# hidasib/GRU4Rec

Measured on AMD Instinct MI355X. Metric: mini-batches/sec (gru4rec.py:661), RSC15-shaped batch=128 n_sample=2048 BPR-max, higher is better.
Workload: dtype f32

## Files before the change

gru4rec_amd/csrc/g4r_eval_kernels.cuh:

```cuda
#pragma once
#include "g4r_step_kernels.cuh"

#define SC_BM 128
#define SC_KC 128

template <int TN, bool COUNT = false>
__global__ __launch_bounds__(256) void k_score_all(const DevModel* __restrict__ mp, const float* h, int mrows, const int* item_idx,
                                                   long long n_sel, float* out, long long ldo, int apply_act,
                                                   int* cnt = nullptr, long long col_begin = 0, const int* tie_col = nullptr,
                                                   unsigned tie_ctr = 0) {
    extern __shared__ __attribute__((aligned(16))) float smem[];
    const DevModel& m = *mp;
    const int tid = threadIdx.x, lane = tid & 63, wid = tid >> 6, li = lane & 15, lg = lane >> 4;
    const int D = m.Dtop;
    const int ldk = SC_KC + 2;
    float* sA = smem;
    float* sB = sA + SC_BM * ldk;
    int* sItem = reinterpret_cast<int*>(sB + TN * ldk);
    const long long n0 = (long long)blockIdx.x * TN;
    const int rbase = blockIdx.y * SC_BM;
    if (tid < TN) {
        const long long n = n0 + tid;
        int item = -1;
        if (n < n_sel) item = item_idx ? item_idx[n] : (int)n;
// ... 182 lines not shown

__global__ void k_selftest_mfma32(const float* A, const float* Bm, float* C, int K) {
    const int lane = threadIdx.x & 63, l32 = lane & 31, lh = lane >> 5;
    f32x16 acc;
    for (int j = 0; j < 16; ++j) acc[j] = 0.f;
    for (int k = 0; k < K; k += 2) acc = mfma32(A[l32 * K + k + lh], Bm[(k + lh) * 32 + l32], acc);
    for (int r = 0; r < 16; ++r) C[(8 * (r >> 2) + 4 * lh + (r & 3)) * 32 + l32] = acc[r];
}

template __global__ void k_sparse_update<1, false>(const DevModel*, StepState*, int);
template __global__ void k_sparse_update<1, true>(const DevModel*, StepState*, int);
template __global__ void k_sparse_update<2, false>(const DevModel*, StepState*, int);
template __global__ void k_sparse_update<2, true>(const DevModel*, StepState*, int);
template __global__ void k_sparse_update_generic<1>(const DevModel*, StepState*, int, int);
template __global__ void k_sparse_update_generic<2>(const DevModel*, StepState*, int, int);
template __global__ void k_loss_rows<false, 0, 1>(const DevModel*, StepState*);
template __global__ void k_loss_rows<false, 0, 4>(const DevModel*, StepState*);
template __global__ void k_loss_rows<false, 1, 1>(const DevModel*, StepState*);
template __global__ void k_loss_rows<false, 1, 4>(const DevModel*, StepState*);
template __global__ void k_loss_rows<false, 2, 1>(const DevModel*, StepState*);
template __global__ void k_loss_rows<false, 2, 4>(const DevModel*, StepState*);
template __global__ void k_loss_rows<false, 3, 1>(const DevModel*, StepState*);
template __global__ void k_loss_rows<false, 3, 4>(const DevModel*, StepState*);
template __global__ void k_loss_rows<true, 0, 4>(const DevModel*, StepState*);
template __global__ void k_loss_rows<true, 1, 4>(const DevModel*, StepState*);
template __global__ void k_loss_rows<true, 2, 4>(const DevModel*, StepState*);
template __global__ void k_loss_rows<true, 3, 4>(const DevModel*, StepState*);
template __global__ void k_sparse_update<4, false>(const DevModel*, StepState*, int);
template __global__ void k_sparse_update<4, true>(const DevModel*, StepState*, int);
template __global__ void k_sparse_update_generic<4>(const DevModel*, StepState*, int, int);
template __global__ void k_update<1, 32, false>(const DevModel*, StepState*, const DenseTile*, int, int);
template __global__ void k_update<1, 32, true>(const DevModel*, StepState*, const DenseTile*, int, int);
template __global__ void k_update<2, 32, false>(const DevModel*, StepState*, const DenseTile*, int, int);
template __global__ void k_update<2, 32, true>(const DevModel*, StepState*, const DenseTile*, int, int);
template __global__ void k_dense_grad<32>(const DevModel*, StepState*, const DenseTile*);
template __global__ void k_score_fwd<GT_BN, GT_BK>(const DevModel*, StepState*);
template __global__ void k_score_fwd<32, 64>(const DevModel*, StepState*);
template __global__ void k_score_fwd<64, 32, T2_BK>(const DevModel*, StepState*);
template __global__ void k_score_fwd<64, 32, 3>(const DevModel*, StepState*);
template __global__ void k_score_bwd<32, GT_BK>(const DevModel*, StepState*, int, int, int, int);
template __global__ void k_score_bwd<64, 64>(const DevModel*, StepState*, int, int, int, int);
template __global__ void k_gru_p1<GT_BN, P1_BK>(const DevModel*, StepState*, int, int, int, GruFwdPredict);
// ... 8 lines not shown
```

gru4rec_amd/csrc/g4r_host_debug.hpp:

```cpp
int g4r_get_debug(g4r_model* m, const char* name, float* host, int64_t count) {
    if (!m || !name || !host) return fail("null argument");
    HIPCHK(hipSetDevice(m->cfg.device));
    DevModel& d = m->dm;
    const StepKernels& k = m->kern;
    std::string s(name);
    const float* p = nullptr; int64_t n = 0;
    int l = 0;
    if (!s.empty() && isdigit((unsigned char)s.back())) { l = s.back() - '0'; s.pop_back(); }
    if (l >= d.n_layers) return fail("layer out of range");
    const int64_t bd = (int64_t)d.B * d.D[l];
    if (s == "scores") { p = d.Sc; n = (int64_t)d.B * d.ldSc; }
    else if (s == "dSx") { p = d.dSx + (size_t)((m->gstep - 1) & d.defer_mask) * (size_t)d.dSx_stride; n = (int64_t)d.B * d.Ein; }
    else if (s == "dSy") { p = d.dSy + (size_t)((m->gstep - 1) & d.defer_mask) * (size_t)d.dSy_stride; n = (int64_t)d.ldSc * d.Dtop; }
    else if (s == "dSBy") { p = d.dSBy + (size_t)((m->gstep - 1) & d.defer_mask) * (size_t)d.dSBy_stride; n = d.ldSc; }
    else if (s == "defer_stats") {
        if (count < 4) return fail("count");
        double rows = 0, bias = 0;
        if (m->defer_on) {
            std::vector<unsigned> st(2048);
            HIPCHK(hipStreamSynchronize(m->stream));
            HIPCHK(hipMemcpy(st.data(), d.dstat, st.size() * sizeof(unsigned), hipMemcpyDeviceToHost));
            for (size_t i = 0; i < st.size(); i += 2) { rows += st[i]; bias += st[i + 1]; }
        }
        host[0] = (float)rows; host[1] = (float)bias; host[2] = m->defer_on ? 1.f : 0.f; host[3] = (float)(d.defer_mask + 1);
// ... 10 lines not shown
        host[1] = (m->sim_valid[0] || m->sim_valid[1]) ? 1.f : 0.f; host[2] = (float)m->sim_builds;
        return 0;
    }
    else if (s == "continue_steps") {
        if (count < 2) return fail("count");
        host[0] = (float)m->ro_calls; host[1] = (float)m->ro_steps;
        return 0;
    }
    else if (s == "events_launches") {
        if (count < 4) return fail("count");
        host[0] = (float)m->ev_steps; host[1] = (float)m->ev_scans; host[2] = (float)m->ev_launches; host[3] = (float)m->ev_pieces;
        return 0;
    }
    else if (s == "dhpart") { p = d.dhpart; n = (int64_t)d.ksplit * d.B * d.Dtop; }
    else if (s == "lossrow") { p = d.lossrow; n = d.B; }
    else if (s == "hd") { p = d.hd[l]; n = bd; }
    else if (s == "r") { p = d.r[l]; n = bd; }
    else if (s == "z") { p = d.z[l]; n = bd; }
    else if (s == "c") { p = d.c[l]; n = bd; }
    else if (s == "Hr") { p = d.Hr[l]; n = bd; }
    else if (s == "dV") { p = d.dV[l]; n = bd * 3; }
    else if (s == "dyl") { p = d.dyl[l]; n = bd; }
    else if (s == "Hprev") { p = d.H[l][(m->gstep + 1) & 1]; n = bd; }
    else if (s == "occ_idx") { p = (const float*)d.occ_idx; n = d.R; }
    else if (s == "own_pos") {
        if (!d.own_pos) return fail("no owner table (k_update_l not chosen, or G4R_OWNER_SCAN=1)");
        p = (const float*)(d.own_pos + (m->own_window ? (size_t)m->own_last * d.R * 16 : (size_t)0)); n = 16 * (int64_t)d.R;
    }
    else if (s == "own_pos_ring") { if (!d.own_pos) return fail("no owner table (k_update_l not chosen, or G4R_OWNER_SCAN=1)"); p = (const float*)d.own_pos; n = (int64_t)G4R_OWN_SLOTS * 16 * d.R; }
    else if (s == "owner_window") { if (count < 1) return fail("count"); host[0] = (m->own_window && k.update == UP_LEAN) ? 1.f : 0.f; return 0; }
// ... 63 lines not shown
}

int g4r_debug_loss_rows(g4r_model* m, float* scores, int64_t count, int32_t M, float* lossrow) {
    if (!m || !scores || !lossrow) return fail("null argument");
    DevModel& d = m->dm;
    if (count != (int64_t)d.B * d.ldSc) return fail("size mismatch for the score rows: expected " + std::to_string((int64_t)d.B * d.ldSc));
    if (M < 1 || M > d.B) return fail("M outside [1, batch_size]");
    HIPCHK(hipSetDevice(m->cfg.device));
    HIPCHK(hipStreamSynchronize(m->stream));
    StepState saved, mine;
    HIPCHK(hipMemcpy(&saved, (const void*)d.st, sizeof(saved), hipMemcpyDeviceToHost));
    HIPCHK(hipMemcpy((void*)d.Sc, scores, (size_t)count * sizeof(float), hipMemcpyHostToDevice));
    mine = saved;
    mine.M_b = M;
    HIPCHK(hipMemcpy((void*)d.st, &mine, sizeof(mine), hipMemcpyHostToDevice));
    StepLauncher lk(m, nullptr);
    launch_loss_rows(lk, dim3(d.B));
    hipError_t e = hipGetLastError();
    if (e == hipSuccess) e = hipStreamSynchronize(m->stream);
    const hipError_t r = hipMemcpy((void*)d.st, &saved, sizeof(saved), hipMemcpyHostToDevice);
    if (e != hipSuccess) return fail(std::string("k_loss_rows: ") + hipGetErrorString(e));
    if (r != hipSuccess) return fail(std::string("step state: ") + hipGetErrorString(r));
    HIPCHK(hipMemcpy(scores, (const void*)d.Sc, (size_t)count * sizeof(float), hipMemcpyDeviceToHost));
    HIPCHK(hipMemcpy(lossrow, (const void*)d.lossrow, (size_t)d.B * sizeof(float), hipMemcpyDeviceToHost));
    return 0;
}

int g4r_debug_gumbel(g4r_model* m, uint64_t seed, uint32_t row_id, uint32_t step, const int32_t* items, int64_t n, float* out) {
    if (!m || !items || !out) return fail("null argument");
    if (n < 1) return fail("n must be positive");
    for (int64_t p = 0; p < n; ++p)
        if (items[p] < 0) return fail("item index out of range");
    HIPCHK(hipSetDevice(m->cfg.device));
    CallTemps tmp(m);
    int* d_it = nullptr;
// ... 132 lines not shown
```

gru4rec_amd/csrc/g4r_host_step.hpp:

```cpp
extern "C++" {
struct StepLauncher {
    g4r_model* m;
    hipStream_t s;
    std::vector<EvRec>* recs;
    size_t evi = 0;
    int kn = -1;
    hipEvent_t ev_a = nullptr, ev_b = nullptr;
    StepLauncher(g4r_model* m_, std::vector<EvRec>* recs_) : m(m_), s(m_->stream), recs(recs_) {}
    void use(int kn_, hipEvent_t a, hipEvent_t b) { kn = kn_; ev_a = a; ev_b = b; }
    void open(int kn_) {
        if (m->sw.trace) { fprintf(stderr, "[g4r] launch %s\n", KN_NAMES[kn_]); fflush(stderr); }
        use(kn_, nullptr, nullptr);
        if (!recs) return;
        while (m->evs.size() < evi + 2) { hipEvent_t e; (void)hipEventCreate(&e); m->evs.push_back(e); }
        use(kn_, m->evs[evi], m->evs[evi + 1]);
        evi += 2;
        recs->push_back(EvRec{kn_, ev_a, ev_b});
    }
    bool skipped() const { return m->sw.skip_kn && kn >= 0 && ((m->sw.skip_kn >> kn) & 1ull); }
    template <class... P, class... A>
    void launch(void (*kern)(P...), dim3 grid, dim3 block, size_t smem, A... a) {
        if (skipped()) return;
        if (ev_a) hipExtLaunchKernelGGL(kern, grid, block, (unsigned)smem, s, ev_a, ev_b, 0, static_cast<P>(a)...);
        else hipLaunchKernelGGL(kern, grid, block, smem, s, static_cast<P>(a)...);
    }
    void close() {
        if (!m->sw.trace) return;
        hipError_t e = hipStreamSynchronize(s);
        fprintf(stderr, "[g4r] done   %s: %s\n", KN_NAMES[kn], hipGetErrorString(e));
        fflush(stderr);
    }
};
}

static void launch_loss_rows(StepLauncher& lk, dim3 grid) {
    g4r_model* m = lk.m;
    lk.launch(loss_rows_kernel(m->kern), grid, dim3(LOSS_T), m->smem_loss, (const DevModel*)m->d_dm, (StepState*)m->dm.st);
}

static inline bool update_merged(const g4r_model* m, const StepLauncher& lk) { return m->kern.update != UP_SPLIT && !(lk.recs && m->profile_split); }

static void gru_forward(g4r_model* m, StepLauncher& lk, int l) {
    const DevModel& d = m->dm;
    const StepKernels& k = m->kern;
    const int B = d.B, first = l == 0 ? 1 : 0;
    const DevModel* dmp = (const DevModel*)m->d_dm;
    StepState* stp = (StepState*)d.st;
    const GruFwdPredict nopa = {};
    if (k.fwd[l] == FWD_LEAN) {
        const dim3 g(cdiv(d.D[l], 16), cdiv(B, 16));
        const LeanV& v = m->h_leanV[l];
        const LeanH& h = m->h_leanH[l];
// ... 257 lines not shown
        HIPCHK(hipMemcpyAsync(Hc, m->d_tmpH, (size_t)B * W * sizeof(float), hipMemcpyDeviceToDevice, m->stream));
    }
    return 0;
}
static int between_steps(g4r_model* m, int64_t t, size_t* ci) {
    while (*ci < m->compact_steps.size() && m->compact_steps[*ci] == t) { if (apply_compaction(m, (int64_t)*ci)) return -1; ++*ci; }
    if (m->dm.ns > 0 && !m->store_frozen && m->gstep > 0 && m->gstep % m->gl == 0) {
        if (refill_store(m)) return -1;
        hipLaunchKernelGGL(k_restage_inputs, dim3(1), dim3(512), 0, m->stream, (const DevModel*)m->d_dm, (StepState*)m->dm.st);
    }
    return 0;
}

#define G4R_GRAPH_STEPS 16
#define G4R_GRAPH_STEPS_SMALL 4
static int capture_steps(g4r_model* m, int n, hipStreamCaptureMode cmode, hipGraphExec_t* out) {
    hipGraph_t graph = nullptr;
    HIPCHK(hipStreamBeginCapture(m->stream, cmode));
    int rc = 0;
    for (int i = 0; i < n && !rc; ++i) rc = whole_step(m, i);
    hipError_t e = hipStreamEndCapture(m->stream, &graph);
    if (rc || e != hipSuccess || !graph) {
        if (graph) (void)hipGraphDestroy(graph);
        (void)hipGetLastError();
        if (!rc) fail(std::string("graph capture: ") + hipGetErrorString(e));
        return -1;
    }
    e = hipGraphInstantiate(out, graph, nullptr, nullptr, 0);
    (void)hipGraphDestroy(graph);
    if (e != hipSuccess) { *out = nullptr; (void)hipGetLastError(); return fail(std::string("graph instantiate: ") + hipGetErrorString(e)); }
    return 0;
}
static int ensure_graph(g4r_model* m) {
    if (m->gexec) return 0;
// ... 29 lines not shown
    if (dist_graph_wanted(m)) {
        if (ensure_graph(m) == 0) return 0;
        m->dist_graph_failed = true;
        fprintf(stderr, "[g4r] RCCL all-reduce could not be captured into the step graph (%s); launching it eagerly\n", g_err.c_str());
    }
    return ensure_head_graph(m);
}

struct StepWindow {
    g4r_model* m;
    const bool own_win;
    bool scanned = false;
    explicit StepWindow(g4r_model* m_) : m(m_), own_win(m_->own_window && m_->kern.update == UP_LEAN && !(m_->profiling && m_->profile_split)) {}
    ~StepWindow() { if (scanned) m->defer_broken = true; }
    bool on() const { return m->defer_on || own_win; }
    int open(int64_t t, int64_t g, int64_t nw) {
        const DevModel& d = m->dm;
        const DevModel* dmp = (const DevModel*)m->d_dm;
        if (own_win) {
            StepLauncher lk(m, nullptr);
            if (m->profiling) for (auto& e : m->ev_ow) if (!e) (void)hipEventCreate(&e);
            lk.use(KN_OWNER_WINDOW, m->profiling ? m->ev_ow[0] : nullptr, m->profiling ? m->ev_ow[1] : nullptr);
            lk.launch(k_owner_window, dim3((unsigned)(nw * cdiv(2 * d.B, OW_NW))), dim3(OW_T), (size_t)(((d.R + 3) & ~3) + 16 * OW_NW) * sizeof(int), dmp, t, g, nw);
            HIPCHK(hipGetLastError());
        }
        if (!m->defer_on) return 0;
        scanned = true;
        const dim3 gs(cdiv(nw * d.R, 256));
        if (m->profiling) (void)hipEventRecord(m->ev_df[0], m->stream);
        hipLaunchKernelGGL(k_defer_scan, gs, dim3(256), 0, m->stream, dmp, (long long)t, (long long)g, (int)nw, 0);
        hipLaunchKernelGGL(k_defer_scan, gs, dim3(256), 0, m->stream, dmp, (long long)t, (long long)g, (int)nw, 1);
        if (m->profiling) (void)hipEventRecord(m->ev_df[1], m->stream);
        return 0;
    }
    int close(int64_t g, int64_t nw) {
        auto timed = [&](int kn, hipEvent_t a, hipEvent_t b) {
            float ms = 0.f;
            if (hipEventElapsedTime(&ms, a, b) == hipSuccess) { m->kn_ms[kn] += ms; m->kn_n[kn]++; }
// ... 70 lines not shown
        }
        int64_t run = tend - t;
        if (devsync) run = std::min<int64_t>(run, m->sync_every_dev - m->since_sync);
        if (ci < m->compact_steps.size()) run = std::min(run, m->compact_steps[ci] - t);
        if (m->dm.ns > 0 && !m->store_frozen) run = std::min<int64_t>(run, m->gl - (m->gstep % m->gl));
        if (run <= 0) return fail("internal: empty run");
        const bool replay = mode == STEP_GRAPH && run >= G4R_GRAPH_STEPS_SMALL;
        if (replay && ensure_graph(m)) return -1;
        for (int64_t done = 0, nw; done < run; done += nw) {
            const int64_t left = run - done;
            hipGraphExec_t g = nullptr;
            if (replay && left >= m->graph_steps) { g = m->gexec; nw = m->graph_steps; }
            else if (replay && m->gexec_small && left >= G4R_GRAPH_STEPS_SMALL) { g = m->gexec_small; nw = G4R_GRAPH_STEPS_SMALL; }
            else nw = win.on() ? std::min<int64_t>(G4R_DEFER_SLOTS, left) : 1;
            const bool windowed = g || win.on();
            if (windowed && win.open(t + done, m->gstep + done, nw)) return -1;
            if (g) HIPCHK(hipGraphLaunch(g, m->stream));
            else for (int i = 0; i < nw; ++i) if (single_step(m, single, windowed ? i : 0, recs)) return -1;
            if (windowed && win.close(m->gstep + done, nw)) return -1;
        }
        t += run;
        m->gstep += run;
        m->since_sync += run;
    }
    HIPCHK(hipStreamSynchronize(m->stream));
    if (m->p2p_ready) {
        unsigned late = 0;
        HIPCHK(hipMemcpy(&late, m->p2p_round + m->p2p_nblk, sizeof(late), hipMemcpyDeviceToHost));
        if (late) return fail("p2p all-reduce: a peer did not publish its gradients within G4R_P2P_TIMEOUT_MS (dead rank?)");
    }
    return 0;
// ... 118 lines not shown
```

gru4rec_amd/csrc/g4r_lean_kernels.cuh:

```cuda
#pragma once

#define LN_MAXD 128

__device__ __forceinline__ float ldu(const GAS float* base, unsigned boff) { return *(const GAS float*)((const GAS char*)base + boff); }
__device__ __forceinline__ int ldu_i(const GAS int* base, unsigned boff) { return *(const GAS int*)((const GAS char*)base + boff); }
__device__ __forceinline__ float4 ldu4(const GAS float* base, unsigned boff) { return *(const GAS float4*)((const GAS char*)base + boff); }
__device__ __forceinline__ void stu(GAS float* base, unsigned boff, float v) { *(GAS float*)((GAS char*)base + boff) = v; }
__device__ __forceinline__ void stu4(GAS float* base, unsigned boff, float4 v) { *(GAS float4*)((GAS char*)base + boff) = v; }

#if defined(G4R_CLK_TRACE)
#define LCLK_INIT(dbgp, slot) GAS long long* clk_ = ((dbgp) && blockIdx.x == 1 && blockIdx.y == 1 && blockIdx.z == 0 && threadIdx.x == 0) ? (dbgp) + (slot) : nullptr
#define LCLK(i) do { if (clk_) clk_[i] = wall_clock64(); } while (0)
#define LCLK_USE(x) do { if (clk_ && (x) == 123.456f) clk_[15] = 0; } while (0)
#define LSPAN_BEGIN(tilep, base) GAS long long* span_ = ((tilep) && threadIdx.x == 0) ? (tilep) + 8 * (size_t)((base) + (blockIdx.z * gridDim.y + blockIdx.y) * gridDim.x + blockIdx.x) : nullptr; \
    if (span_) span_[0] = wall_clock64()
#define LSPAN_END() do { if (span_) span_[1] = wall_clock64(); } while (0)
#define LSPAN_BEGIN_AT(tilep, idx, lead) GAS long long* span_ = ((tilep) && (lead)) ? (tilep) + 8 * (size_t)(idx) : nullptr; \
    if (span_) span_[0] = wall_clock64()
#else
#define LCLK_INIT(dbgp, slot)
#define LCLK(i)
#define LCLK_USE(x)
#define LSPAN_BEGIN(tilep, base)
#define LSPAN_END()
// ... 63 lines not shown
};

struct LeanU {
    const DevModel* mp; StepState* st;
    GP(float) Wy; GP(float) E; GP(float) accWy; GP(float) accE; GP(float) velWy; GP(float) velE;
    GP(float) By; GP(float) accBy; GP(float) velBy;
    GP(const float) dAx; GP(const float) dAy; GP(const float) dABy;
    GP(float) dense_p; GP(float) dense_acc; GP(float) dense_vel; GP(const float) yin0;
    GP(const int) meta;
    GP(long long) dbg; GP(long long) dbgtile;
    int n_items, constrained, wE, wY;
    float lr, mom, lmbd, pad;
    int own_on, pad2;
};

template <typename T> __device__ __forceinline__ void lean_pin1(T v) {
#if defined(__HIP_DEVICE_COMPILE__)
    asm volatile("" ::"s"(v));
#endif
}
template <typename... T> __device__ __forceinline__ void lean_pin(T... v) { (lean_pin1(v), ...); }
__device__ __forceinline__ void lean_keep(float& x) {
#if defined(__HIP_DEVICE_COMPILE__)
    asm volatile("" : "+v"(x));
#endif
}
struct LeanState { unsigned g; int M; unsigned t_lo; };
__device__ __forceinline__ LeanState lean_state(int4 mt) {
    LeanState s;
    s.g = (unsigned)__builtin_amdgcn_readfirstlane(mt.x); s.M = __builtin_amdgcn_readfirstlane(mt.z); s.t_lo = (unsigned)__builtin_amdgcn_readfirstlane(mt.w);
    return s;
}

template <bool L0, bool DROPE>
__global__ __launch_bounds__(512) void k_gru_v(const LeanV* __restrict__ ap, StepState* st_, const int* cur_in_, const float* Wx_, const float* Wrz_,
                                               const float* H0_, const float* H1_, unsigned dims, unsigned B) {
    __shared__ float sJ[4 * 8 * 64];
    const unsigned tid = threadIdx.x, lane = tid & 63, li = lane & 15, lg = lane >> 4;
    const unsigned wid = __builtin_amdgcn_readfirstlane(tid >> 6);
    const unsigned part = blockIdx.z, m0 = blockIdx.y * 16, rowA = m0 + li;
    const unsigned D = dims & 0xFFFFu, IN = dims >> 16;
    const GAS float *Wx = (const GAS float*)Wx_, *Wrz = (const GAS float*)Wrz_, *H0 = (const GAS float*)H0_, *H1 = (const GAS float*)H1_;
    const GAS int* cur_in = (const GAS int*)cur_in_;
    const unsigned rowB = min(rowA, B - 1);
    int item = 0;
    if (L0) item = ldu_i(cur_in, 4u * rowB);
    const int4 mt = ldi4(cur_in + 2 * B);
    const unsigned ncol = 16 * blockIdx.x + li, nc = min(ncol, D - 1);
// ... 941 lines not shown
```

gru4rec_amd/csrc/g4r_loss_kernel.cuh:

```cuda
#pragma once
#ifndef LOSS_T
#define LOSS_T 1024
#endif
#define LOSS_NW (LOSS_T / 64)
template <int NV, bool MAX>
__device__ __forceinline__ void block_reduce(float (&v)[NV], float* red) {
    const int lane = threadIdx.x & 63, w = threadIdx.x >> 6;
#pragma unroll
    for (int q = 0; q < NV; ++q) v[q] = MAX ? wave_max(v[q]) : wave_sum(v[q]);
    if (lane == 0) {
#pragma unroll
        for (int q = 0; q < NV; ++q) red[q * LOSS_NW + w] = v[q];
    }
    __syncthreads();
#pragma unroll
    for (int q = 0; q < NV; ++q) {
        float a = red[q * LOSS_NW];
#pragma unroll
        for (int u = 1; u < LOSS_NW; ++u) a = MAX ? fmaxf(a, red[q * LOSS_NW + u]) : a + red[q * LOSS_NW + u];
        v[q] = a;
    }
}

__device__ __forceinline__ float softplusf_(float x) {
// ... 49 lines not shown
                cnt += __popcll(mk[e]);
            }
#pragma unroll
            for (int e = 0; e < 4; ++e) {
                if ((mk[e] >> lane) & 1ull) {
                    if ((unsigned)at < (unsigned)G4R_OWN_INLINE) pos[1 + at] = j0 + e;
                    ++at;
                }
            }
        }
    }
    if (lane == 0) pos[0] = min(cnt, G4R_OWN_INLINE);
}

template <bool LONG_ROW, int SPEC, int V>
__global__ __launch_bounds__(LOSS_T) void k_loss_rows(const DevModel* __restrict__ mp, StepState* st) {
    const DevModel& m = *mp;
    extern __shared__ __attribute__((aligned(16))) float smem[];
    const int tid = threadIdx.x;
    const int B = m.B, N = m.N, i = blockIdx.x;
    const int fact = SPEC == 1 || SPEC == 3 ? (int)G4R_ACT_ELU : (SPEC == 2 ? (int)G4R_ACT_SOFTMAX : m.final_act);
    const int lossk = SPEC == 1 ? (int)G4R_LOSS_BPR_MAX : (SPEC == 2 ? (int)G4R_LOSS_XE : (SPEC == 3 ? (int)G4R_LOSS_TOP1_MAX : m.loss));
    const int ldSc = m.ldSc;
    const float fp0 = m.fa_p0, fp1 = m.fa_p1, invB = m.inv_B, bpreg = m.bpreg, smooth = m.smoothing;
    GAS float* row = m.Sc + (size_t)i * ldSc;
    float* sy = smem;
    std::conditional_t<LONG_ROW, GAS float*, float*> se;
    if constexpr (LONG_ROW) se = row; else se = smem + ldSc;
    float* red = smem + (LONG_ROW ? 1 : 2) * ldSc;
    constexpr int STEP = V * LOSS_T;
    const int jt = V * tid;
    constexpr int LOSS_PRE = (V == 4) ? 2 : 4;
#if defined(G4R_CLK_TRACE)
    struct Span { GAS long long* p; __device__ ~Span() { if (p) p[1] = wall_clock64(); } } span_{(m.dbgtile && tid == 0 && i < 532) ? m.dbgtile + 8 * (size_t)(7168 + i) : nullptr};
    if (span_.p) span_.p[0] = wall_clock64();
#endif
    const StepCtx c = load_ctx(st);
    if (i >= B) {
        const unsigned nown = gridDim.x - B, R = m.R;
        for (unsigned k = (threadIdx.x >> 6) * nown + (unsigned)(i - B); k < R; k += LOSS_NW * nown) owner_prescan(m, k);
        return;
    }
    float pre_s[LOSS_PRE][V];
#pragma unroll
    for (int q = 0; q < LOSS_PRE; ++q) vld<V>(pre_s[q], row + min(jt + q * STEP, ldSc - V));
    const int M = c.M;
    if (i >= M) return;
    const bool fsm = (fact == G4R_ACT_SOFTMAX), fsl = (fact == G4R_ACT_SOFTMAX_LOGIT);
    const float n_out = (float)(M + (N - B));
    auto active = [&](int j) { return j < N && (j < M || j >= B); };
    auto grp_fast = [&](int j0) { return (j0 >= B && j0 + V <= N) || (j0 + V <= G4R_MUT_FAST_M(M) && (i < j0 || i >= j0 + V)); };
    using Fast = std::true_type;
    using Slow = std::false_type;
#define G4R_GROUPS(lim, fn) for (int j0 = jt; j0 < (lim); j0 += STEP) { if (grp_fast(j0)) fn(Fast{}, j0); else fn(Slow{}, j0); }
    float mneg[1] = {0.f};
    if (fsm || fsl) {
        float mx[1] = {-INFINITY};
        auto first = [&](auto F, int j0, const float (&v)[V]) {
            float o[V];
#pragma unroll
            for (int e = 0; e < V; ++e) {
// ... 74 lines not shown
    if (lossk == G4R_LOSS_XE && fsm && smooth == 0.f) {
        Lrow = -logf(yd + G4R_EPS_LOSS);
        const float coef = yd / (yd + G4R_EPS_LOSS);
        auto grad = [&](auto F, int j0) {
            float y[V], o[V];
            vld<V>(y, sy + j0);
#pragma unroll
            for (int e = 0; e < V; ++e) {
                const int j = j0 + e;
                if (F.value) o[e] = coef * y[e] * invB;
                else o[e] = active(j) ? coef * (y[e] - (j == i ? 1.f : 0.f)) * invB : 0.f;
            }
            vst<V>(row + j0, o);
        };
        G4R_GROUPS(ldSc, grad)
        if (tid == 0) m.lossrow[i] = Lrow;
        return;
    }
    if (lossk == G4R_LOSS_XE || lossk == G4R_LOSS_XE_LOGIT) {
        const bool lg = (lossk == G4R_LOSS_XE_LOGIT);
        const float wd = 1.f - n_out / (n_out - 1.f) * smooth, wa = smooth / (n_out - 1.f);
        float sa[1] = {0.f};
        for (int j0 = jt; j0 < N; j0 += STEP) {
            float y[V], d[V];
            vld<V>(y, sy + j0);
#pragma unroll
            for (int e = 0; e < V; ++e) {
                const int j = j0 + e;
                const bool a = active(j);
                const float yy = a ? y[e] : 1.f;
                float dd = 0.f;
// ... 105 lines not shown
                vld<V>(y, sy + j0);
                vld<V>(ev, se + j0);
#pragma unroll
                for (int e = 0; e < V; ++e) {
                    const int j = j0 + e;
                    if (F.value) o[e] = dLn(y[e], ev[e]) * act_bwd_from_out(fact, fp0, fp1, y[e]) * invB;
                    else {
                        const bool a = active(j);
                        const float yy = a ? y[e] : 0.f, ex = a ? ev[e] : 0.f;
                        o[e] = a ? dL(j, yy, ex) * act_bwd_from_out(fact, fp0, fp1, yy) * invB : 0.f;
                    }
                }
                vst<V>(row + j0, o);
            };
            G4R_GROUPS(ldSc, grad)
            if (tid == 0) m.lossrow[i] = Lrow;
            return;
        }
        for (int j0 = jt; j0 < N; j0 += STEP) {
            float y[V], ev[V];
            vld<V>(y, sy + j0);
            vld<V>(ev, se + j0);
#pragma unroll
            for (int e = 0; e < V; ++e) {
                const bool a = active(j0 + e);
                ev[e] = dL(j0 + e, a ? y[e] : 0.f, a ? ev[e] : 0.f);
            }
            vst<V>(se + j0, ev);
        }
    }
    float inner[1] = {0.f};
// ... 12 lines not shown
        vld<V>(y, sy + j0);
        vld<V>(d, se + j0);
#pragma unroll
        for (int e = 0; e < V; ++e) {
            const bool a = F.value || active(j0 + e);
            const float yy = a ? y[e] : 0.f, dd = a ? d[e] : 0.f;
            float out;
            if (fsm) out = yy * (dd - inner[0]);
            else if (fsl) out = fexp(-yy) * inner[0] - dd;
            else out = dd * act_bwd_from_out(fact, fp0, fp1, yy);
            o[e] = a ? out * invB : 0.f;
        }
        vst<V>(row + j0, o);
    };
    G4R_GROUPS(ldSc, grad)
    if (tid == 0) m.lossrow[i] = Lrow;
#undef G4R_GROUPS
}
```

gru4rec_amd/csrc/g4r_step_kernels.cuh:

```cuda
#pragma once
#include <type_traits>

#include "g4r_gemm.cuh"

struct StepCtx { long long t, g; int M; };

__device__ __forceinline__ StepCtx load_ctx_first(StepState* st_) {
    GAS StepState* st = (GAS StepState*)st_;
    StepCtx c;
    c.t = st->t_a; c.g = st->g_a; c.M = st->M_a;
    if (blockIdx.x == 0 && blockIdx.y == 0 && threadIdx.x == 0) { st->t_b = c.t; st->g_b = c.g; st->M_b = c.M; }
    return c;
}
__device__ __forceinline__ StepCtx load_ctx(StepState* st_) {
    const GAS StepState* st = (const GAS StepState*)st_;
    StepCtx c;
    c.t = st->t_b; c.g = st->g_b; c.M = st->M_b;
    return c;
}

__device__ __forceinline__ void stage_step_inputs(const DevModel& m, long long t, long long g, int M, int tid, int nth) {
    const int B = m.B, N = m.N, ld = m.ldSc;
    const GAS int* in = m.in_idx + t * B;
    const GAS int* out = m.out_idx + t * B;
    const GAS int* smp = m.ST + (size_t)(m.gl > 0 ? g % m.gl : 0) * m.ns;
    GAS int *ci = m.cur_in, *cc = m.cur_col;
    const GAS unsigned char* rst = m.reset + t * B;
    for (int b = tid; b < B; b += nth) { ci[b] = in[b]; ci[B + b] = rst[b]; }
    if (tid == 0) { ci[2 * B] = (int)(unsigned)g; ci[2 * B + 1] = (int)(g >> 32); ci[2 * B + 2] = M; ci[2 * B + 3] = (int)(unsigned)t; ci[2 * B + 4] = (int)(t >> 32); }
    for (int base = 0; base < ld; base += 8 * nth) {
        int vo[8], vs[8];
#pragma unroll
        for (int q = 0; q < 8; ++q) {
// ... 86 lines not shown
```

gru4rec_amd/csrc/g4r_update_kernels.cuh:

```cuda
#pragma once
__global__ __launch_bounds__(256) void k_onehot_step(const DevModel* __restrict__ mp, StepState* st) {
    const DevModel& m = *mp;
    const StepCtx c = load_ctx(st);
    const int W = m.Ein, nc4 = W >> 2;
    const long long q = (long long)blockIdx.x * 256 + threadIdx.x;
    const int row = (int)(q / nc4), c4 = (int)(q % nc4);
    if (row >= c.M) return;
    const int item = m.occ_idx[row];
    if (item < 0) return;
    const float lr = m.lr;
    const float4 g = ld4(m.dV[0] + (size_t)row * W + 4 * c4);
    const float4 a = ld4(m.accE + (size_t)item * W + 4 * c4);
    const int cnt = m.occ_fl[4 * ((size_t)m.n_items + item) + 2];
    const float4 an = make_float4(a.x + g.x * g.x, a.y + g.y * g.y, a.z + g.z * g.z, a.w + g.w * g.w);
    if (!m.generic && cnt == 1) st4(m.accE + (size_t)item * W + 4 * c4, an);
    else st4(m.dAx + (size_t)row * W + 4 * c4, an);
    if (m.generic) { st4(G4R_DSX(m, c.g) + (size_t)row * W + 4 * c4, g); return; }
    st4(G4R_DSX(m, c.g) + (size_t)row * W + 4 * c4, make_float4(lr * g.x * frsq(an.x + G4R_EPS_ADAGRAD), lr * g.y * frsq(an.y + G4R_EPS_ADAGRAD),
                                                         lr * g.z * frsq(an.z + G4R_EPS_ADAGRAD), lr * g.w * frsq(an.w + G4R_EPS_ADAGRAD)));
}

struct DenseTile {
    GP(const float) X0; GP(const float) X1; GP(const float) dV;
    long long base;
// ... 506 lines not shown
    const long long idx = (long long)blockIdx.x * 256 + threadIdx.x;
    const int R = m.R, s = (int)(idx / R), k = (int)(idx - (long long)s * R);
    if (s >= n) return;
    int table;
    const int item = defer_item(m, t0 + s, g0 + s, k, table);
    const size_t slot = G4R_SLOT(m, g0 + s) * (size_t)m.dRcap + k;
    if (item < 0) { if (pass) m.dcand[slot] = 0; return; }
    GAS int* lu = m.last_use + (size_t)table * m.n_items + item;
    if (pass == 0) atomicMax((int*)lu, (int)(g0 + s));
    else m.dcand[slot] = (*lu == (int)(g0 + s)) ? 1 : 0;
}
#define OW_T 1024
#define OW_NW (OW_T / 64)
static_assert(G4R_OWN_INLINE + 1 == 16, "an owner-table row is 16 ints: the count and G4R_OWN_INLINE positions");
static_assert(((size_t)G4R_OWN_WINDOW_MAXR + 16 * OW_NW) * sizeof(int) <= 65536, "k_owner_window: the longest list and the waves' position rows share one workgroup's 64 KB of LDS");
__global__ __launch_bounds__(OW_T) void k_owner_window(const DevModel* __restrict__ mp, long long t0, long long g0, int nw) {
    const DevModel& m = *mp;
    extern __shared__ __attribute__((aligned(16))) int sid[];
    const int R = m.R, B = m.B, Rp = (R + 3) & ~3;
    const int gps = (2 * B + OW_NW - 1) / OW_NW;
    const int s = (int)blockIdx.x / gps, q = (int)blockIdx.x - s * gps;
#if defined(G4R_CLK_TRACE)
    struct Span { GAS long long* p; __device__ ~Span() { if (p) p[1] = wall_clock64(); } } span_{(m.dbgtile && threadIdx.x == 0 && blockIdx.x < 400) ? m.dbgtile + 8 * (size_t)(7700 + blockIdx.x) : nullptr};
    if (span_.p) span_.p[0] = wall_clock64();
#endif
    if (s >= nw) return;
    for (int k = threadIdx.x; k < Rp; k += OW_T) {
        int table;
        sid[k] = k < R ? defer_item(m, t0 + s, G4R_MUT_WIN_G(g0, s), k, table) : -1;
    }
    __syncthreads();
    const int lane = threadIdx.x & 63, wid = threadIdx.x >> 6;
    const int p = q * OW_NW + wid;
    if (p >= 2 * B) return;
    const int item = sid[p];
    if (item < 0) return;
    const bool constrained = m.embed_mode == G4R_EMBED_CONSTRAINED;
    const int ta = (constrained || p < B) ? 0 : B, tb = (!constrained && p < B) ? B : R;
    int* spos = sid + Rp + 16 * wid;
    const unsigned long long below = (1ull << lane) - 1ull;
    int cnt = 0, last = p;
    for (int base0 = ta & ~3; base0 < tb; base0 += 1024) {
        int4 vv[4];
#pragma unroll
// ... 31 lines not shown
                    ++at;
                }
                cnt += __popcll(mk[e]);
            }
        }
    }
    if (cnt < 2) return;
    GAS int* pos = m.own_pos + ((size_t)s * (size_t)R + (size_t)last) * 16;
    if (cnt - 1 > G4R_OWN_INLINE) {
        if (lane == 0) pos[0] = -1;
        return;
    }
    __builtin_amdgcn_fence(__ATOMIC_ACQ_REL, "wavefront");
    if (lane < cnt - 1) pos[1 + lane] = spos[lane];
    if (lane == 0) pos[0] = cnt - 1;
}
#define FL_NR 4
__global__ __launch_bounds__(SP_WAVES * 64) void k_sparse_flush(const DevModel* __restrict__ mp, long long g0, int n) {
    const DevModel& m = *mp;
    const int lane = threadIdx.x & 63, wid = threadIdx.x >> 6;
    const long long e0 = ((long long)blockIdx.x * SP_WAVES + wid) * FL_NR;
    const int Rc = m.dRcap, s = (int)(e0 / Rc), k0 = (int)(e0 - (long long)s * Rc);
    if (s >= n) return;
    const size_t slot = G4R_SLOT(m, g0 + s) * (size_t)Rc + k0;
    int it[FL_NR];
#pragma unroll
    for (int u = 0; u < FL_NR; ++u) it[u] = m.dlist[slot + u];
    if (lane < FL_NR) { m.dcand[slot + lane] = 0; m.dlist[slot + lane] = -1; }
    const int B = m.B;
    const bool sep = m.embed_mode != G4R_EMBED_CONSTRAINED;
// ... 384 lines not shown
```

Baseline: 27010.

## Capture owner-window kernel inside step graph and streamline loss kernel prologue

The owner-window scan is now launched inside the captured step graph, using a device-side variant that reads the window start from the step state, so graph replays no longer need a separate host launch per window. The owner-window staging loop inlines item lookup with batched loads in place of per-element defer_item calls. The loss kernel takes Sc, the step metadata and the dimensions as kernel arguments and issues its row prefetch before loading model fields, reading M from the metadata block rather than the StepState. This adds graph-capture complexity and depends on t_a/g_a and the metadata being correct at replay time.

```diff
diff --git a/gru4rec_amd/csrc/g4r_eval_kernels.cuh b/gru4rec_amd/csrc/g4r_eval_kernels.cuh
--- a/gru4rec_amd/csrc/g4r_eval_kernels.cuh
+++ b/gru4rec_amd/csrc/g4r_eval_kernels.cuh
@@ -220,18 +220,18 @@
 template __global__ void k_sparse_update<2, true>(const DevModel*, StepState*, int);
 template __global__ void k_sparse_update_generic<1>(const DevModel*, StepState*, int, int);
 template __global__ void k_sparse_update_generic<2>(const DevModel*, StepState*, int, int);
-template __global__ void k_loss_rows<false, 0, 1>(const DevModel*, StepState*);
-template __global__ void k_loss_rows<false, 0, 4>(const DevModel*, StepState*);
-template __global__ void k_loss_rows<false, 1, 1>(const DevModel*, StepState*);
-template __global__ void k_loss_rows<false, 1, 4>(const DevModel*, StepState*);
-template __global__ void k_loss_rows<false, 2, 1>(const DevModel*, StepState*);
-template __global__ void k_loss_rows<false, 2, 4>(const DevModel*, StepState*);
-template __global__ void k_loss_rows<false, 3, 1>(const DevModel*, StepState*);
-template __global__ void k_loss_rows<false, 3, 4>(const DevModel*, StepState*);
-template __global__ void k_loss_rows<true, 0, 4>(const DevModel*, StepState*);
-template __global__ void k_loss_rows<true, 1, 4>(const DevModel*, StepState*);
-template __global__ void k_loss_rows<true, 2, 4>(const DevModel*, StepState*);
-template __global__ void k_loss_rows<true, 3, 4>(const DevModel*, StepState*);
+template __global__ void k_loss_rows<false, 0, 1>(const DevModel*, StepState*, float*, const int*, int, int, int);
+template __global__ void k_loss_rows<false, 0, 4>(const DevModel*, StepState*, float*, const int*, int, int, int);
+template __global__ void k_loss_rows<false, 1, 1>(const DevModel*, StepState*, float*, const int*, int, int, int);
+template __global__ void k_loss_rows<false, 1, 4>(const DevModel*, StepState*, float*, const int*, int, int, int);
+template __global__ void k_loss_rows<false, 2, 1>(const DevModel*, StepState*, float*, const int*, int, int, int);
+template __global__ void k_loss_rows<false, 2, 4>(const DevModel*, StepState*, float*, const int*, int, int, int);
+template __global__ void k_loss_rows<false, 3, 1>(const DevModel*, StepState*, float*, const int*, int, int, int);
+template __global__ void k_loss_rows<false, 3, 4>(const DevModel*, StepState*, float*, const int*, int, int, int);
+template __global__ void k_loss_rows<true, 0, 4>(const DevModel*, StepState*, float*, const int*, int, int, int);
+template __global__ void k_loss_rows<true, 1, 4>(const DevModel*, StepState*, float*, const int*, int, int, int);
+template __global__ void k_loss_rows<true, 2, 4>(const DevModel*, StepState*, float*, const int*, int, int, int);
+template __global__ void k_loss_rows<true, 3, 4>(const DevModel*, StepState*, float*, const int*, int, int, int);
 template __global__ void k_sparse_update<4, false>(const DevModel*, StepState*, int);
 template __global__ void k_sparse_update<4, true>(const DevModel*, StepState*, int);
 template __global__ void k_sparse_update_generic<4>(const DevModel*, StepState*, int, int);
diff --git a/gru4rec_amd/csrc/g4r_host_debug.hpp b/gru4rec_amd/csrc/g4r_host_debug.hpp
--- a/gru4rec_amd/csrc/g4r_host_debug.hpp
+++ b/gru4rec_amd/csrc/g4r_host_debug.hpp
@@ -48,6 +48,8 @@
     }
     else if (s == "dhpart") { p = d.dhpart; n = (int64_t)d.ksplit * d.B * d.Dtop; }
     else if (s == "lossrow") { p = d.lossrow; n = d.B; }
+    else if (s == "step_state") { p = (const float*)d.st; n = (int64_t)(sizeof(StepState) / sizeof(float)); }
+    else if (s == "step_meta") { p = (const float*)(d.cur_in + 2 * d.B); n = 5; }
     else if (s == "hd") { p = d.hd[l]; n = bd; }
     else if (s == "r") { p = d.r[l]; n = bd; }
     else if (s == "z") { p = d.z[l]; n = bd; }
@@ -141,11 +143,20 @@
     mine = saved;
     mine.M_b = M;
     HIPCHK(hipMemcpy((void*)d.st, &mine, sizeof(mine), hipMemcpyHostToDevice));
+    int* const meta_M = (int*)d.cur_in + 2 * d.B + 2;
+    int saved_M = 0;
+    HIPCHK(hipMemcpy(&saved_M, meta_M, sizeof(int), hipMemcpyDeviceToHost));
+    if (hipMemcpy(meta_M, &M, sizeof(int), hipMemcpyHostToDevice) != hipSuccess) {
+        (void)hipMemcpy((void*)d.st, &saved, sizeof(saved), hipMemcpyHostToDevice);
+        return fail("staged step state: copy failed");
+    }
     StepLauncher lk(m, nullptr);
     launch_loss_rows(lk, dim3(d.B));
     hipError_t e = hipGetLastError();
     if (e == hipSuccess) e = hipStreamSynchronize(m->stream);
-    const hipError_t r = hipMemcpy((void*)d.st, &saved, sizeof(saved), hipMemcpyHostToDevice);
+    hipError_t r = hipMemcpy((void*)d.st, &saved, sizeof(saved), hipMemcpyHostToDevice);
+    const hipError_t r2 = hipMemcpy(meta_M, &saved_M, sizeof(int), hipMemcpyHostToDevice);
+    if (r == hipSuccess) r = r2;
     if (e != hipSuccess) return fail(std::string("k_loss_rows: ") + hipGetErrorString(e));
     if (r != hipSuccess) return fail(std::string("step state: ") + hipGetErrorString(r));
     HIPCHK(hipMemcpy(scores, (const void*)d.Sc, (size_t)count * sizeof(float), hipMemcpyDeviceToHost));
diff --git a/gru4rec_amd/csrc/g4r_host_step.hpp b/gru4rec_amd/csrc/g4r_host_step.hpp
--- a/gru4rec_amd/csrc/g4r_host_step.hpp
+++ b/gru4rec_amd/csrc/g4r_host_step.hpp
@@ -35,7 +35,8 @@
 
 static void launch_loss_rows(StepLauncher& lk, dim3 grid) {
     g4r_model* m = lk.m;
-    lk.launch(loss_rows_kernel(m->kern), grid, dim3(LOSS_T), m->smem_loss, (const DevModel*)m->d_dm, (StepState*)m->dm.st);
+    const DevModel& d = m->dm;
+    lk.launch(loss_rows_kernel(m->kern), grid, dim3(LOSS_T), m->smem_loss, (const DevModel*)m->d_dm, (StepState*)d.st, d.Sc, d.cur_in + 2 * d.B, d.B, d.N, d.ldSc);
 }
 
 static inline bool update_merged(const g4r_model* m, const StepLauncher& lk) { return m->kern.update != UP_SPLIT && !(lk.recs && m->profile_split); }
@@ -323,10 +324,24 @@
 
 #define G4R_GRAPH_STEPS 16
 #define G4R_GRAPH_STEPS_SMALL 4
+static inline bool owner_windows(const g4r_model* m) { return m->own_window && m->kern.update == UP_LEAN; }
+static void launch_owner_window(g4r_model* m, StepLauncher& lk, int64_t nw, const StepState* st, int64_t t, int64_t g) {
+    const DevModel& d = m->dm;
+    const DevModel* dmp = (const DevModel*)m->d_dm;
+    const dim3 grid((unsigned)(nw * cdiv(2 * d.B, OW_NW)));
+    const size_t smem = (size_t)(((d.R + 3) & ~3) + 16 * OW_NW) * sizeof(int);
+    if (st) lk.launch(k_owner_window_dev, grid, dim3(OW_T), smem, dmp, st, nw);
+    else lk.launch(k_owner_window, grid, dim3(OW_T), smem, dmp, t, g, nw);
+}
 static int capture_steps(g4r_model* m, int n, hipStreamCaptureMode cmode, hipGraphExec_t* out) {
     hipGraph_t graph = nullptr;
     HIPCHK(hipStreamBeginCapture(m->stream, cmode));
     int rc = 0;
+    if (owner_windows(m)) {
+        StepLauncher lk(m, nullptr);
+        lk.use(KN_OWNER_WINDOW, nullptr, nullptr);
+        launch_owner_window(m, lk, n, (const StepState*)m->dm.st, 0, 0);
+    }
     for (int i = 0; i < n && !rc; ++i) rc = whole_step(m, i);
     hipError_t e = hipStreamEndCapture(m->stream, &graph);
     if (rc || e != hipSuccess || !graph) {
@@ -386,14 +401,14 @@
     explicit StepWindow(g4r_model* m_) : m(m_), own_win(m_->own_window && m_->kern.update == UP_LEAN && !(m_->profiling && m_->profile_split)) {}
     ~StepWindow() { if (scanned) m->defer_broken = true; }
     bool on() const { return m->defer_on || own_win; }
-    int open(int64_t t, int64_t g, int64_t nw) {
+    int open(int64_t t, int64_t g, int64_t nw, bool replay) {
         const DevModel& d = m->dm;
         const DevModel* dmp = (const DevModel*)m->d_dm;
-        if (own_win) {
+        if (own_win && !replay) {
             StepLauncher lk(m, nullptr);
             if (m->profiling) for (auto& e : m->ev_ow) if (!e) (void)hipEventCreate(&e);
             lk.use(KN_OWNER_WINDOW, m->profiling ? m->ev_ow[0] : nullptr, m->profiling ? m->ev_ow[1] : nullptr);
-            lk.launch(k_owner_window, dim3((unsigned)(nw * cdiv(2 * d.B, OW_NW))), dim3(OW_T), (size_t)(((d.R + 3) & ~3) + 16 * OW_NW) * sizeof(int), dmp, t, g, nw);
+            launch_owner_window(m, lk, nw, nullptr, t, g);
             HIPCHK(hipGetLastError());
         }
         if (!m->defer_on) return 0;
@@ -494,7 +509,7 @@
             else if (replay && m->gexec_small && left >= G4R_GRAPH_STEPS_SMALL) { g = m->gexec_small; nw = G4R_GRAPH_STEPS_SMALL; }
             else nw = win.on() ? std::min<int64_t>(G4R_DEFER_SLOTS, left) : 1;
             const bool windowed = g || win.on();
-            if (windowed && win.open(t + done, m->gstep + done, nw)) return -1;
+            if (windowed && win.open(t + done, m->gstep + done, nw, g != nullptr)) return -1;
             if (g) HIPCHK(hipGraphLaunch(g, m->stream));
             else for (int i = 0; i < nw; ++i) if (single_step(m, single, windowed ? i : 0, recs)) return -1;
             if (windowed && win.close(m->gstep + done, nw)) return -1;
diff --git a/gru4rec_amd/csrc/g4r_lean_kernels.cuh b/gru4rec_amd/csrc/g4r_lean_kernels.cuh
--- a/gru4rec_amd/csrc/g4r_lean_kernels.cuh
+++ b/gru4rec_amd/csrc/g4r_lean_kernels.cuh
@@ -101,24 +101,11 @@
     int own_on, pad2;
 };
 
-template <typename T> __device__ __forceinline__ void lean_pin1(T v) {
-#if defined(__HIP_DEVICE_COMPILE__)
-    asm volatile("" ::"s"(v));
-#endif
-}
-template <typename... T> __device__ __forceinline__ void lean_pin(T... v) { (lean_pin1(v), ...); }
 __device__ __forceinline__ void lean_keep(float& x) {
 #if defined(__HIP_DEVICE_COMPILE__)
     asm volatile("" : "+v"(x));
 #endif
 }
-struct LeanState { unsigned g; int M; unsigned t_lo; };
-__device__ __forceinline__ LeanState lean_state(int4 mt) {
-    LeanState s;
-    s.g = (unsigned)__builtin_amdgcn_readfirstlane(mt.x); s.M = __builtin_amdgcn_readfirstlane(mt.z); s.t_lo = (unsigned)__builtin_amdgcn_readfirstlane(mt.w);
-    return s;
-}
-
 template <bool L0, bool DROPE>
 __global__ __launch_bounds__(512) void k_gru_v(const LeanV* __restrict__ ap, StepState* st_, const int* cur_in_, const float* Wx_, const float* Wrz_,
                                                const float* H0_, const float* H1_, unsigned dims, unsigned B) {
diff --git a/gru4rec_amd/csrc/g4r_loss_kernel.cuh b/gru4rec_amd/csrc/g4r_loss_kernel.cuh
--- a/gru4rec_amd/csrc/g4r_loss_kernel.cuh
+++ b/gru4rec_amd/csrc/g4r_loss_kernel.cuh
@@ -87,37 +87,41 @@
 }
 
 template <bool LONG_ROW, int SPEC, int V>
-__global__ __launch_bounds__(LOSS_T) void k_loss_rows(const DevModel* __restrict__ mp, StepState* st) {
-    const DevModel& m = *mp;
+__global__ __launch_bounds__(LOSS_T) void k_loss_rows(const DevModel* __restrict__ mp, StepState* st, float* Sc_, const int* meta_, int B, int N, int ldSc) {
     extern __shared__ __attribute__((aligned(16))) float smem[];
     const int tid = threadIdx.x;
-    const int B = m.B, N = m.N, i = blockIdx.x;
+    const int i = blockIdx.x;
+    (void)st;
+    if (i >= B) {
+        const DevModel& m = *mp;
+        const unsigned nown = gridDim.x - B, R = m.R;
+        for (unsigned k = (threadIdx.x >> 6) * nown + (unsigned)(i - B); k < R; k += LOSS_NW * nown) owner_prescan(m, k);
+        return;
+    }
+    GAS float* row = (GAS float*)Sc_ + (size_t)i * ldSc;
+    constexpr int STEP = V * LOSS_T;
+    const int jt = V * tid;
+    constexpr int LOSS_PRE = (V == 4) ? 2 : 4;
+    float pre_s[LOSS_PRE][V];
+#pragma unroll
+    for (int q = 0; q < LOSS_PRE; ++q) vld<V>(pre_s[q], row + min(jt + q * STEP, ldSc - V));
+    const int4 mt = ldi4((const GAS int*)meta_);
+    const DevModel& m = *mp;
     const int fact = SPEC == 1 || SPEC == 3 ? (int)G4R_ACT_ELU : (SPEC == 2 ? (int)G4R_ACT_SOFTMAX : m.final_act);
     const int lossk = SPEC == 1 ? (int)G4R_LOSS_BPR_MAX : (SPEC == 2 ? (int)G4R_LOSS_XE : (SPEC == 3 ? (int)G4R_LOSS_TOP1_MAX : m.loss));
-    const int ldSc = m.ldSc;
     const float fp0 = m.fa_p0, fp1 = m.fa_p1, invB = m.inv_B, bpreg = m.bpreg, smooth = m.smoothing;
-    GAS float* row = m.Sc + (size_t)i * ldSc;
+    GAS float* const lossrow = m.lossrow;
+    if constexpr (SPEC == 0) lean_pin(fact, lossk);
+    lean_pin(fp0, fp1, invB, bpreg, smooth, lossrow);
+#if defined(G4R_CLK_TRACE)
+    struct Span { GAS long long* p; __device__ ~Span() { if (p) p[1] = wall_clock64(); } } span_{(m.dbgtile && tid == 0 && i < 532) ? m.dbgtile + 8 * (size_t)(7168 + i) : nullptr};
+    if (span_.p) span_.p[0] = wall_clock64();
+#endif
     float* sy = smem;
     std::conditional_t<LONG_ROW, GAS float*, float*> se;
     if constexpr (LONG_ROW) se = row; else se = smem + ldSc;
     float* red = smem + (LONG_ROW ? 1 : 2) * ldSc;
-    constexpr int STEP = V * LOSS_T;
-    const int jt = V * tid;
-    constexpr int LOSS_PRE = (V == 4) ? 2 : 4;
-#if defined(G4R_CLK_TRACE)
-    struct Span { GAS long long* p; __device__ ~Span() { if (p) p[1] = wall_clock64(); } } span_{(m.dbgtile && tid == 0 && i < 532) ? m.dbgtile + 8 * (size_t)(7168 + i) : nullptr};
-    if (span_.p) span_.p[0] = wall_clock64();
-#endif
-    const StepCtx c = load_ctx(st);
-    if (i >= B) {
-        const unsigned nown = gridDim.x - B, R = m.R;
-        for (unsigned k = (threadIdx.x >> 6) * nown + (unsigned)(i - B); k < R; k += LOSS_NW * nown) owner_prescan(m, k);
-        return;
-    }
-    float pre_s[LOSS_PRE][V];
-#pragma unroll
-    for (int q = 0; q < LOSS_PRE; ++q) vld<V>(pre_s[q], row + min(jt + q * STEP, ldSc - V));
-    const int M = c.M;
+    const int M = lean_state(mt).M;
     if (i >= M) return;
     const bool fsm = (fact == G4R_ACT_SOFTMAX), fsl = (fact == G4R_ACT_SOFTMAX_LOGIT);
     const float n_out = (float)(M + (N - B));
@@ -222,7 +226,7 @@
             vst<V>(row + j0, o);
         };
         G4R_GROUPS(ldSc, grad)
-        if (tid == 0) m.lossrow[i] = Lrow;
+        if (tid == 0) lossrow[i] = Lrow;
         return;
     }
     if (lossk == G4R_LOSS_XE || lossk == G4R_LOSS_XE_LOGIT) {
@@ -358,7 +362,7 @@
                 vst<V>(row + j0, o);
             };
             G4R_GROUPS(ldSc, grad)
-            if (tid == 0) m.lossrow[i] = Lrow;
+            if (tid == 0) lossrow[i] = Lrow;
             return;
         }
         for (int j0 = jt; j0 < N; j0 += STEP) {
@@ -401,6 +405,6 @@
         vst<V>(row + j0, o);
     };
     G4R_GROUPS(ldSc, grad)
-    if (tid == 0) m.lossrow[i] = Lrow;
+    if (tid == 0) lossrow[i] = Lrow;
 #undef G4R_GROUPS
 }
diff --git a/gru4rec_amd/csrc/g4r_step_kernels.cuh b/gru4rec_amd/csrc/g4r_step_kernels.cuh
--- a/gru4rec_amd/csrc/g4r_step_kernels.cuh
+++ b/gru4rec_amd/csrc/g4r_step_kernels.cuh
@@ -17,6 +17,19 @@
     StepCtx c;
     c.t = st->t_b; c.g = st->g_b; c.M = st->M_b;
     return c;
+}
+
+template <typename T> __device__ __forceinline__ void lean_pin1(T v) {
+#if defined(__HIP_DEVICE_COMPILE__)
+    asm volatile("" ::"s"(v));
+#endif
+}
+template <typename... T> __device__ __forceinline__ void lean_pin(T... v) { (lean_pin1(v), ...); }
+struct LeanState { unsigned g; int M; unsigned t_lo; };
+__device__ __forceinline__ LeanState lean_state(int4 mt) {
+    LeanState s;
+    s.g = (unsigned)__builtin_amdgcn_readfirstlane(mt.x); s.M = __builtin_amdgcn_readfirstlane(mt.z); s.t_lo = (unsigned)__builtin_amdgcn_readfirstlane(mt.w);
+    return s;
 }
 
 __device__ __forceinline__ void stage_step_inputs(const DevModel& m, long long t, long long g, int M, int tid, int nth) {
diff --git a/gru4rec_amd/csrc/g4r_update_kernels.cuh b/gru4rec_amd/csrc/g4r_update_kernels.cuh
--- a/gru4rec_amd/csrc/g4r_update_kernels.cuh
+++ b/gru4rec_amd/csrc/g4r_update_kernels.cuh
@@ -544,9 +544,7 @@
 #define OW_NW (OW_T / 64)
 static_assert(G4R_OWN_INLINE + 1 == 16, "an owner-table row is 16 ints: the count and G4R_OWN_INLINE positions");
 static_assert(((size_t)G4R_OWN_WINDOW_MAXR + 16 * OW_NW) * sizeof(int) <= 65536, "k_owner_window: the longest list and the waves' position rows share one workgroup's 64 KB of LDS");
-__global__ __launch_bounds__(OW_T) void k_owner_window(const DevModel* __restrict__ mp, long long t0, long long g0, int nw) {
-    const DevModel& m = *mp;
-    extern __shared__ __attribute__((aligned(16))) int sid[];
+__device__ __forceinline__ void owner_window_body(const DevModel& m, long long t0, long long g0, int nw, int* sid) {
     const int R = m.R, B = m.B, Rp = (R + 3) & ~3;
     const int gps = (2 * B + OW_NW - 1) / OW_NW;
     const int s = (int)blockIdx.x / gps, q = (int)blockIdx.x - s * gps;
@@ -555,9 +553,29 @@
     if (span_.p) span_.p[0] = wall_clock64();
 #endif
     if (s >= nw) return;
-    for (int k = threadIdx.x; k < Rp; k += OW_T) {
-        int table;
-        sid[k] = k < R ? defer_item(m, t0 + s, G4R_MUT_WIN_G(g0, s), k, table) : -1;
+    {
+        const long long t = t0 + s, g = G4R_MUT_WIN_G(g0, s);
+        const int M = m.Mplan[t], ns = m.ns;
+        const GAS int *in = m.in_idx + t * B, *out = m.out_idx + t * B;
+        const GAS int* smp = ns > 0 ? m.ST + (size_t)(m.gl > 0 ? g % m.gl : 0) * ns : in;
+        for (int base = 0; base < Rp; base += 4 * OW_T) {
+            int vx[4], vy[4], vs[4];
+#pragma unroll
+            for (int q = 0; q < 4; ++q) {
+                const int k = base + q * OW_T + (int)threadIdx.x;
+                vx[q] = in[min(k, B - 1)];
+                vy[q] = out[min(max(k - B, 0), B - 1)];
+                vs[q] = smp[min(max(k - 2 * B, 0), max(ns, 1) - 1)];
+            }
+            __builtin_amdgcn_sched_barrier(0);
+#pragma unroll
+            for (int q = 0; q < 4; ++q) {
+                const int k = base + q * OW_T + (int)threadIdx.x;
+                const int item = k < B ? vx[q] : (k < 2 * B ? vy[q] : vs[q]);
+                const bool on = k < B ? k < M : (k < 2 * B ? k - B < M : M > 0);
+                if (k < Rp) sid[k] = (k < R && on) ? item : -1;
+            }
+        }
     }
     __syncthreads();
     const int lane = threadIdx.x & 63, wid = threadIdx.x >> 6;
@@ -619,6 +637,17 @@
     __builtin_amdgcn_fence(__ATOMIC_ACQ_REL, "wavefront");
     if (lane < cnt - 1) pos[1 + lane] = spos[lane];
     if (lane == 0) pos[0] = cnt - 1;
+}
+__global__ __launch_bounds__(OW_T) void k_owner_window(const DevModel* __restrict__ mp, long long t0, long long g0, int nw) {
+    extern __shared__ __attribute__((aligned(16))) int sid[];
+    owner_window_body(*mp, t0, g0, nw, sid);
+}
+__global__ __launch_bounds__(OW_T) void k_owner_window_dev(const DevModel* __restrict__ mp, const StepState* st, int nw) {
+    extern __shared__ __attribute__((aligned(16))) int sid[];
+    const GAS StepState* sg = (const GAS StepState*)st;
+    const long long t0 = sg->t_a, g0 = sg->g_a;
+    lean_pin(t0, g0);
+    owner_window_body(*mp, t0, g0, nw, sid);
 }
 #define FL_NR 4
 __global__ __launch_bounds__(SP_WAVES * 64) void k_sparse_flush(const DevModel* __restrict__ mp, long long g0, int n) {
```

Result: no change. 27170 (median of 6 runs) (+0.6%).
